# fpthink/PDGN

Measured on AMD Instinct MI355X. Metric: generator+D step points/sec (B=35, 256->2048 pts), higher is better.
Workload: dtype f32; 1 GPU; PDGNet_v2 G+D iteration (models/PDGNet_v2.py:171-256), chair-shaped synthetic batch, per-GPU batch 35, 256->2048 pts, random-init weights; global_batch=35, parallelism=dp1, losses_finite=True, hipgraph=False, issue=list

## Files before the change

### include/pdgn_hip.h

```cpp
#ifndef PDGN_HIP_H
#define PDGN_HIP_H

#include <stdint.h>

#ifdef __cplusplus
extern "C" {
#endif

#define PDGN_ERR_INVALID (-1)
#define PDGN_KNN_MAX_NSAMPLE 200

typedef void *pdgn_stream_t;

#define PDGN_ABI_VERSION 35
int pdgn_abi_version(void);

int pdgn_knnquery(int b, int n, int m, int nsample, const float *xyz, const float *new_xyz,
                  int32_t *idx, float *dist2, pdgn_stream_t stream);

int pdgn_grouping_forward(int b, int c, int n, int m, int nsample, const float *points,
                          const int32_t *idx, float *out, pdgn_stream_t stream);

int pdgn_grouping_backward(int b, int c, int n, int m, int nsample, const float *grad_out,
                           const int32_t *idx, float *grad_points, pdgn_stream_t stream);

int pdgn_nearestneighbor(int b, int n, int m, const float *unknown, const float *known,
                         float *dist2, int32_t *idx, pdgn_stream_t stream);

int pdgn_interpolation_forward(int b, int c, int m, int n, const float *points,
                               const int32_t *idx, const float *weight, float *out,
                               pdgn_stream_t stream);

int pdgn_interpolation_backward(int b, int c, int n, int m, const float *grad_out,
                                const int32_t *idx, const float *weight, float *grad_points,
                                pdgn_stream_t stream);

int pdgn_nndistance(int b, int n, const float *xyz, int m, const float *xyz2, float *result,
                    int32_t *result_i, float *result2, int32_t *result2_i, pdgn_stream_t stream);

int pdgn_nndistance_grad(int b, int n, const float *xyz1, int m, const float *xyz2,
                         const float *grad_dist1, const int32_t *idx1, const float *grad_dist2,
                         const int32_t *idx2, float *grad_xyz1, float *grad_xyz2,
                         pdgn_stream_t stream);

int pdgn_approxmatch(int b, int n, int m, const float *xyz1, const float *xyz2, float *match,
                     float *temp, pdgn_stream_t stream);

// ... 12 lines not shown

int pdgn_window_gather_sum(int b, int n, int k, int ldy, int T, int P, int C, int off, int offc,
                           const float *Y, const int32_t *idx, const float *bias, int bias_bstride,
                           float *out, pdgn_stream_t stream);
int pdgn_window_gather_sum_stats(int b, int n, int k, int ldy, int T, int P, int C, int off, int offc,
                                 const float *Y, const int32_t *idx, const float *bias, int bias_bstride,
                                 float *out, float *scratch, pdgn_stream_t stream);

int pdgn_window_gather_sum_backward(int b, int n, int k, int ldy, int T, int P, int C, int off,
                                    int offc, const float *dout, const int32_t *idx, float *dY,
                                    pdgn_stream_t stream);

int pdgn_knn_graph_transpose(int b, int n, int k, const int32_t *idx, int32_t *rowptr, int32_t *edges,
                             int32_t *scratch, pdgn_stream_t stream);
int pdgn_window_gather_sum_backward_csr(int b, int n, int k, int ldy, int T, int P, int C, int off,
                                        int offc, const float *dout, const int32_t *rowptr,
                                        const int32_t *edges, float *dY, unsigned *max_out, int max_init, pdgn_stream_t stream);

long long pdgn_bn_scratch_floats(long long rows, int c);
int pdgn_bn_stats(long long rows, int c, float eps, float momentum, const float *x, const float *gamma,
                  const float *beta, const float *pre_bias, float *running_mean, float *running_var,
                  float *scratch, float *stats, pdgn_stream_t stream);
int pdgn_bn_eval_stats(int c, float eps, const float *gamma, const float *beta, const float *pre_bias,
                       const float *running_mean, const float *running_var, float *stats,
                       pdgn_stream_t stream);
int pdgn_bn_stats_from_partials(long long rows, int c, float eps, float momentum, const float *gamma,
                                const float *beta, const float *pre_bias, float *running_mean, float *running_var,
                                const float *scratch, float *stats, pdgn_stream_t stream);
int pdgn_bn_stats_from_gemm_partials(long long rows, int c, long long nparts, int block_rows, float eps, float momentum,
                                     const float *gamma, const float *beta, const float *pre_bias,
                                     float *running_mean, float *running_var, const float *partials,
                                     float *stats, double *scratch, pdgn_stream_t stream);
long long pdgn_bn_blocks_scratch_doubles(int c, long long nparts);
int pdgn_bn_act_forward(long long rows, int c, int act, const float *x, const float *stats,
                        const float *mul, float *y, int interleave_n, pdgn_stream_t stream);
int pdgn_bn_act_backward(long long rows, int c, int act, int training, const float *x,
                         const float *dy, const float *mul, const float *stats, float *scratch,
                         float *bsums, float *dx, float *dmul, int interleave_n, pdgn_stream_t stream);

long long pdgn_bn_maxpool_scratch_floats(int b, int c);
int pdgn_bn_act_maxpool(int b, int n, int c, int act, const float *x, const float *stats, float *scratch,
                        float *ymax, int32_t *yarg, pdgn_stream_t stream);
long long pdgn_bn_stats_maxpool_scratch_floats(int b, int c);
int pdgn_bn_stats_act_maxpool(int b, int n, int c, int act, float eps, float momentum, const float *x, const float *gamma,
                              const float *beta, const float *pre_bias, float *running_mean, float *running_var, float *scratch,
                              float *stats, float *ymax, int32_t *yarg, pdgn_stream_t stream);
int pdgn_bn_act_maxpool_backward(int b, int n, int c, int act, int training, const float *x,
                                 const float *dout, const int32_t *yarg, const float *stats,
                                 float *scratch, float *bsums, float *dx, pdgn_stream_t stream);
long long pdgn_dense_bn_maxpool_backward_scratch(int b, int c, int k);
int pdgn_dense_bn_maxpool_backward(int b, int n, int c, int k, int act, const float *x, const float *dout, const int32_t *yarg,
                                   const float *stats, const float *h, int ldh, const float *W, int ldw, float *scratch,
                                   float *dh, float *dW, int lddw, float *bsums, pdgn_stream_t stream);
long long pdgn_dense_bn_maxpool_input_grad_scratch(int b, int c, int k);
int pdgn_dense_bn_maxpool_input_grad(int b, int n, int c, int k, int act, const float *x, const float *dout,
                                     const int32_t *yarg, const float *stats, const float *h, int ldh,
                                     const float *W, int ldw, float *scratch, float *dh, pdgn_stream_t stream);

int pdgn_group_colsum(long long groups, long long group_rows, int c, const float *x, long long ldx, float *out,
                      pdgn_stream_t stream);

int pdgn_softmax_slots_permute(long long m, int k, int c, const float *h, float *w, pdgn_stream_t stream);
int pdgn_bn_softmax_slots_permute(long long m, int k, int c, int act, const float *x, const float *stats,
                                  float *w, pdgn_stream_t stream);
int pdgn_bn_softmax_slots_permute_mul(long long m, int k, int c, int act, const float *x, const float *stats,
                                      int act_u, const float *u, const float *stats_u, float *w, float *y,
// ... 266 lines not shown
```

### pdgn_amd/csrc/bnact.hip

```cpp
#include "common.h"

#include "bn_geom.h"
#define ACT_NONE 0
#define ACT_RELU 1
#define ACT_LEAKY 2

__device__ __forceinline__ float act_fwd(float z, int act) {
    if (act == ACT_RELU) return fmaxf(z, 0.f);
    if (act == ACT_LEAKY) return z > 0.f ? z : 0.01f * z;
    return z;
}
__device__ __forceinline__ float act_grad(float z, int act) {
    if (act == ACT_RELU) return z > 0.f ? 1.f : 0.f;
    if (act == ACT_LEAKY) return z > 0.f ? 1.f : 0.01f;
    return 1.f;
}

struct ClGeom {
    int cg, cgb, rl;
};

__global__ __launch_bounds__(BN_THREADS) void cl_stats_kernel(long long R, int C, int cgb, int rows_per_block,
                                                              const float *__restrict__ x,
                                                              float *__restrict__ part) {
// ... 152 lines not shown
            const double mb = pv + s * inv;
            a += n * mb;
            b += (sq - s * s * inv) + n * mb * mb;
        }
    red[pl][cl] = a;
    red2[pl][cl] = b;
    __syncthreads();
    for (int h = FIN_PL / 2; h > 0; h >>= 1) {
        if (pl < h) {
            red[pl][cl] += red[pl + h][cl];
            red2[pl][cl] += red2[pl + h][cl];
        }
        __syncthreads();
    }
    if (!ok || threadIdx.x >= FIN_CH) return;
    const double mean = red[0][cl] / (double)R;
    double var = red2[0][cl] / (double)R - mean * mean;
    var = var < 0 ? 0 : var;
    const float invstd = (float)(1.0 / sqrt(var + (double)eps));
    const float g = gamma ? gamma[c] : 1.f, be = beta ? beta[c] : 0.f;
    const float scale = g * invstd;
    stats[c] = scale;
    stats[C + c] = be - (float)mean * scale;
    stats[2 * C + c] = (float)mean;
    stats[3 * C + c] = invstd;
    if (running_mean) {
        const double unbiased = R > 1 ? var * (double)R / (double)(R - 1) : var;
        const float mb = (float)mean + (pre_bias ? pre_bias[c] : 0.f);
        running_mean[c] = (1.f - momentum) * running_mean[c] + momentum * mb;
        running_var[c] = (1.f - momentum) * running_var[c] + momentum * (float)unbiased;
    }
}

__global__ __launch_bounds__(FIN_CH * FIN_PL) void cl_finalize_blocks_slice_kernel(
    long long R, int C, int nparts, int rpp, int per_slice, const float *__restrict__ part, double *__restrict__ scratch) {
    __shared__ double red[FIN_PL][FIN_CH], red2[FIN_PL][FIN_CH];
    const int cl = threadIdx.x % FIN_CH, pl = threadIdx.x / FIN_CH;
    const int c = blockIdx.x * FIN_CH + cl;
    const bool ok = c < C;
    double a = 0, b = 0;
    const double inv_full = 1.0 / (double)rpp;
    const int pmax_all = (int)min((long long)nparts, (R + rpp - 1) / rpp);
    const int p0 = blockIdx.y * per_slice, pmax = min(pmax_all, p0 + per_slice);
    if (ok)
#pragma unroll 4
        for (int p = p0 + pl; p < pmax; p += FIN_PL) {
            const long long left = R - (long long)p * rpp;
            const bool full = left >= rpp;
            const double n = (double)(full ? rpp : left), inv = full ? inv_full : 1.0 / (double)left;
            const float *q = part + (size_t)p * 3 * C + c;
            const double s = (double)q[0], sq = (double)q[C], pv = (double)q[2 * C];
            const double mb = pv + s * inv;
            a += n * mb;
            b += (sq - s * s * inv) + n * mb * mb;
        }
    red[pl][cl] = a;
    red2[pl][cl] = b;
    __syncthreads();
    for (int h = FIN_PL / 2; h > 0; h >>= 1) {
        if (pl < h) {
            red[pl][cl] += red[pl + h][cl];
            red2[pl][cl] += red2[pl + h][cl];
        }
        __syncthreads();
    }
    if (!ok || threadIdx.x >= FIN_CH) return;
// ... 38 lines not shown
    __shared__ double ra[4][64], rb[4][64];
    const int cl = threadIdx.x & 63, pl = threadIdx.x >> 6;
    const int c = blockIdx.x * 64 + cl;
    double a = 0, b = 0;
    if (c < C)
        for (int s = pl; s < slices; s += 4) {
            a += scratch[((size_t)s * 2) * C + c];
            b += scratch[((size_t)s * 2 + 1) * C + c];
        }
    ra[pl][cl] = a;
    rb[pl][cl] = b;
    __syncthreads();
    if (pl != 0 || c >= C) return;
    a = ((ra[0][cl] + ra[1][cl]) + ra[2][cl]) + ra[3][cl];
    b = ((rb[0][cl] + rb[1][cl]) + rb[2][cl]) + rb[3][cl];
    const double mean = a / (double)R;
    double var = b / (double)R - mean * mean;
    var = var < 0 ? 0 : var;
    const float invstd = (float)(1.0 / sqrt(var + (double)eps));
    const float g = gamma ? gamma[c] : 1.f, be = beta ? beta[c] : 0.f;
    const float scale = g * invstd;
    stats[c] = scale;
    stats[C + c] = be - (float)mean * scale;
    stats[2 * C + c] = (float)mean;
    stats[3 * C + c] = invstd;
    if (running_mean) {
        const double unbiased = R > 1 ? var * (double)R / (double)(R - 1) : var;
        const float mb = (float)mean + (pre_bias ? pre_bias[c] : 0.f);
        running_mean[c] = (1.f - momentum) * running_mean[c] + momentum * mb;
        running_var[c] = (1.f - momentum) * running_var[c] + momentum * (float)unbiased;
    }
}

static inline int fb_slices(int c, long long nparts) {
    if (nparts < 512) return 0;
    if (c % 64 == 0) {
        if (nparts <= 1400) return 0;
        long long s64 = nparts / 64;
        return (int)(s64 < 2 ? 2 : (s64 > 128 ? 128 : s64));
    }
    long long s = 512 / (c / 4 > 0 ? c / 4 : 1);
    s = s > 32 ? 32 : s;
    while (s > 1 && nparts / s < 128) s >>= 1;
    return s < 2 ? 0 : (int)s;
}

__global__ void cl_eval_stats_kernel(int C, float eps, const float *__restrict__ gamma, const float *__restrict__ beta,
                                     const float *__restrict__ pre_bias, const float *__restrict__ running_mean,
                                     const float *__restrict__ running_var, float *__restrict__ stats) {
    const int c = blockIdx.x * blockDim.x + threadIdx.x;
    if (c >= C) return;
    const float invstd = rsqrtf(running_var[c] + eps);
    const float g = gamma ? gamma[c] : 1.f, b = beta ? beta[c] : 0.f;
    const float m = running_mean[c] - (pre_bias ? pre_bias[c] : 0.f);
    stats[c] = g * invstd;
    stats[C + c] = b - m * g * invstd;
    stats[2 * C + c] = m;
    stats[3 * C + c] = invstd;
}

__device__ __forceinline__ void cl_interleaved_rows(long long r, int pn, long long &ra, long long &rb) {
    const long long b = r / pn;
    ra = b * 2 * pn + (r - b * pn);
    rb = ra + pn;
}

__global__ __launch_bounds__(BN_THREADS) void cl_apply_kernel(long long R, int C, int cgb, int rows_per_block, int act,
                                                              const float *__restrict__ x,
                                                              const float *__restrict__ stats,
                                                              const float *__restrict__ mul, float *__restrict__ y, int pn) {
    const int cgl = threadIdx.x % cgb, rlane = threadIdx.x / cgb, rl = BN_THREADS / cgb;
    const int cgi = blockIdx.x * cgb + cgl;
    if (cgi * 4 >= C) return;
    const long long r0 = (long long)blockIdx.y * rows_per_block;
    const long long r1 = min(R, r0 + rows_per_block);
    const float4 sc = *reinterpret_cast<const float4 *>(stats + cgi * 4);
    const float4 sh = *reinterpret_cast<const float4 *>(stats + C + cgi * 4);
// ... 183 lines not shown

extern "C" int pdgn_bn_stats(long long rows, int c, float eps, float momentum, const float *x, const float *gamma,
                             const float *beta, const float *pre_bias, float *running_mean, float *running_var,
                             float *scratch, float *stats, pdgn_stream_t stream) {
    if (rows < 1 || c < 4 || c % 4) return PDGN_ERR_INVALID;
    hipStream_t s = (hipStream_t)stream;
    int cgb, gx, gy, rpb;
    cl_geometry(rows, c, &cgb, &gx, &gy, &rpb);
    hipLaunchKernelGGL(cl_stats_kernel, dim3(gx, gy), dim3(BN_THREADS), 0, s, rows, c, cgb, rpb, x, scratch);
    hipLaunchKernelGGL(cl_finalize_kernel, dim3(cdiv(c, FIN_CH)), dim3(FIN_CH * FIN_PL), 0, s, rows, c, gy, eps, momentum, scratch,
                       gamma, beta, pre_bias, running_mean, running_var, stats, x);
    return pdgn_launch_status();
}

extern "C" int pdgn_bn_stats_from_partials(long long rows, int c, float eps, float momentum, const float *gamma,
                                           const float *beta, const float *pre_bias, float *running_mean,
                                           float *running_var, const float *scratch, float *stats, pdgn_stream_t stream) {
    if (rows < 1 || c < 4 || c % 4) return PDGN_ERR_INVALID;
    int cgb, gx, gy, rpb;
    cl_geometry(rows, c, &cgb, &gx, &gy, &rpb);
    hipLaunchKernelGGL(cl_finalize_kernel, dim3(cdiv(c, FIN_CH)), dim3(FIN_CH * FIN_PL), 0, (hipStream_t)stream, rows, c, gy, eps,
                       momentum, scratch, gamma, beta, pre_bias, running_mean, running_var, stats, (const float *)nullptr);
    return pdgn_launch_status();
}

extern "C" int pdgn_bn_stats_from_gemm_partials(long long rows, int c, long long nparts, int block_rows, float eps,
                                                float momentum, const float *gamma, const float *beta, const float *pre_bias,
                                                float *running_mean, float *running_var, const float *partials,
                                                float *stats, double *scratch, pdgn_stream_t stream) {
    if (rows < 1 || c < 4 || c % 4 || nparts < 1 || nparts > 0x7fffffffLL || block_rows < 1 ||
        nparts * (long long)block_rows < rows)
        return PDGN_ERR_INVALID;
    const int slices = scratch ? fb_slices(c, nparts) : 0;
    if (slices > 1) {
        const int per = (int)((nparts + slices - 1) / slices);
        if (c % 64 == 0)
            hipLaunchKernelGGL(cl_finalize_blocks_slice64_kernel, dim3(c / 64, slices), dim3(256), 0, (hipStream_t)stream, rows, c, (int)nparts,
                               block_rows, per, partials, scratch);
        else
            hipLaunchKernelGGL(cl_finalize_blocks_slice_kernel, dim3(cdiv(c, FIN_CH), slices), dim3(FIN_CH * FIN_PL), 0,
                               (hipStream_t)stream, rows, c, (int)nparts, block_rows, per, partials, scratch);
        hipLaunchKernelGGL(cl_finalize_blocks_join_kernel, dim3(cdiv(c, 64)), dim3(256), 0, (hipStream_t)stream, rows, c, slices,
                           eps, momentum, (const double *)scratch, gamma, beta, pre_bias, running_mean, running_var, stats);
        return pdgn_launch_status();
    }
    hipLaunchKernelGGL(cl_finalize_blocks_kernel, dim3(cdiv(c, FIN_CH)), dim3(FIN_CH * FIN_PL), 0, (hipStream_t)stream, rows, c,
                       (int)nparts, block_rows, eps, momentum, partials, gamma, beta, pre_bias, running_mean, running_var, stats);
    return pdgn_launch_status();
}

extern "C" long long pdgn_bn_blocks_scratch_doubles(int c, long long nparts) {
    if (c < 1 || nparts < 1) return PDGN_ERR_INVALID;
    return (long long)fb_slices(c, nparts) * 2 * c;
}

extern "C" int pdgn_bn_eval_stats(int c, float eps, const float *gamma, const float *beta, const float *pre_bias,
                                  const float *running_mean, const float *running_var, float *stats,
                                  pdgn_stream_t stream) {
    if (c < 1) return PDGN_ERR_INVALID;
    hipLaunchKernelGGL(cl_eval_stats_kernel, dim3(cdiv(c, 256)), dim3(256), 0, (hipStream_t)stream, c, eps, gamma,
                       beta, pre_bias, running_mean, running_var, stats);
    return pdgn_launch_status();
}

extern "C" int pdgn_bn_act_forward(long long rows, int c, int act, const float *x, const float *stats, const float *mul,
                                   float *y, int interleave_n, pdgn_stream_t stream) {
    if (rows < 1 || c < 4 || c % 4 || act < 0 || act > 2) return PDGN_ERR_INVALID;
    if (interleave_n < 0 || (interleave_n > 0 && (rows % interleave_n || mul))) return PDGN_ERR_INVALID;
    int cgb, gx, gy, rpb;
    cl_geometry(rows, c, &cgb, &gx, &gy, &rpb);
    hipLaunchKernelGGL(cl_apply_kernel, dim3(gx, gy), dim3(BN_THREADS), 0, (hipStream_t)stream, rows, c, cgb, rpb, act,
                       x, stats, mul, y, interleave_n);
    return pdgn_launch_status();
}

extern "C" int pdgn_bn_act_backward(long long rows, int c, int act, int training, const float *x, const float *dy,
                                    const float *mul, const float *stats, float *scratch, float *bsums, float *dx,
                                    float *dmul, int interleave_n, pdgn_stream_t stream) {
    if (rows < 1 || c < 4 || c % 4 || act < 0 || act > 2) return PDGN_ERR_INVALID;
    if (interleave_n < 0 || (interleave_n > 0 && (rows % interleave_n || mul))) return PDGN_ERR_INVALID;
// ... 778 lines not shown
```

### pdgn_amd/csrc/gemm_x3.hip

```cpp
#include <atomic>
#include <type_traits>

#include "gemm_shared.h"

#ifndef X3_FENCE
#define X3_FENCE 2
#endif
#ifndef X3_DEFAULT_MASK
#define X3_DEFAULT_MASK 0x000
#endif
#ifndef X3_FENCE16
#define X3_FENCE16 2
#endif
#ifndef X3_ABLATE
#define X3_ABLATE 0
#endif

typedef float f32x16 __attribute__((ext_vector_type(16)));
typedef float f32x2 __attribute__((ext_vector_type(2)));
typedef __bf16 bf16x8 __attribute__((ext_vector_type(8)));
typedef __bf16 bf16x2 __attribute__((ext_vector_type(2)));

struct X3Parts {
    u32x4 h, m, l;
// ... 17 lines not shown
__device__ __forceinline__ f32x16 x3_mfma(const u32x4 a, const u32x4 b, const f32x16 c) {
    return __builtin_amdgcn_mfma_f32_32x32x16_bf16(__builtin_bit_cast(bf16x8, a), __builtin_bit_cast(bf16x8, b), c, 0, 0, 0);
}

typedef _Float16 f16x8 __attribute__((ext_vector_type(8)));
typedef _Float16 f16x2 __attribute__((ext_vector_type(2)));
__device__ __forceinline__ unsigned x2_cvt_pk(float a, float b) {
    const f32x2 v = {a, b};
    return __builtin_bit_cast(unsigned, __builtin_convertvector(v, f16x2));
}
__device__ __forceinline__ f32x16 x2_mfma(const u32x4 a, const u32x4 b, const f32x16 c) {
    return __builtin_amdgcn_mfma_f32_32x32x16_f16(__builtin_bit_cast(f16x8, a), __builtin_bit_cast(f16x8, b), c, 0, 0, 0);
}
#ifndef X2_PRODUCTS
#define X2_PRODUCTS 3
#endif

typedef float f32x4a __attribute__((ext_vector_type(4)));
__device__ __forceinline__ f32x4a x3_mfma16(const u32x4 a, const u32x4 b, const f32x4a c) {
    return __builtin_amdgcn_mfma_f32_16x16x32_bf16(__builtin_bit_cast(bf16x8, a), __builtin_bit_cast(bf16x8, b), c, 0, 0, 0);
}

template <int MS>
__device__ __forceinline__ unsigned x3_sw(unsigned r) {
    const unsigned x = (r >> 2) & 3u;
    return MS == 32 ? x : ((0x78u >> (2u * x)) & 3u);
}

template <int CTRL, int ROW_MASK>
__device__ __forceinline__ float x3_dpp_add(float v) {
    return v + __int_as_float(__builtin_amdgcn_update_dpp(0, __float_as_int(v), CTRL, ROW_MASK, 0xf, true));
}

__device__ __forceinline__ float x3_half_wave_sum(float v) {
    v = x3_dpp_add<0x111, 0xf>(v);
    v = x3_dpp_add<0x112, 0xf>(v);
    v = x3_dpp_add<0x114, 0xf>(v);
    v = x3_dpp_add<0x118, 0xf>(v);
    return x3_dpp_add<0x142, 0xa>(v);
}

__device__ __forceinline__ float x3_row_sum(float v) {
    v = x3_dpp_add<0x111, 0xf>(v);
    v = x3_dpp_add<0x112, 0xf>(v);
    v = x3_dpp_add<0x114, 0xf>(v);
    return x3_dpp_add<0x118, 0xf>(v);
}

template <int TM, int TN, int WM, int WN, int OCC, bool ATOMIC, bool WT, bool AT, bool EPI = false, bool PW = false, int MS = 32, int NP = 3>
__global__ __launch_bounds__(64 * WM * WN, OCC) void gemm_x3_kernel(const NtArgs p) {
    static_assert(!PW || (!WT && !AT), "pre-split second operand: row-major (N x K) planes only");
    static_assert(MS == 32 || MS == 16, "matrix instruction: 32x32x16 or 16x16x32");
    static_assert(NP == 3 || (NP == 2 && MS == 32), "parts: three bf16, or two fp16 on the 32x32x16 instruction");
    constexpr int NW = WM * WN, NTH = 64 * NW, BM = 32 * TM * WM, BN = 32 * TN * WN;
    constexpr int PART_A = BM * 64, PART_W = BN * 64, STAGE = NP * (PART_A + PART_W);
    constexpr int UNT = NP == 2 ? (BM + BN) * 4 : 0;
    constexpr bool STG = OCC == 1 && !ATOMIC && !(X3_ABLATE & 128) && 2 * STAGE + NW * 4096 + UNT <= 160 * 1024;
    __shared__ __attribute__((aligned(1024))) unsigned char smem[2 * STAGE + (STG ? NW * 4096 : 0) + UNT];
    float *const untab = reinterpret_cast<float *>(smem + 2 * STAGE + (STG ? NW * 4096 : 0));

    const int tid = threadIdx.x, lane = tid & 63;
    const int wave = __builtin_amdgcn_readfirstlane(tid >> 6);
    const int wm = wave / WN, wn = wave % WN;
    const int li = MS == 32 ? lane & 31 : lane & 15, lg = MS == 32 ? lane >> 5 : lane >> 4;

    const int G = gridDim.x, pid = blockIdx.x;
    const int gq = G >> 3, gr = G & 7, xcd = pid & 7;
    const int v = xcd * gq + min(xcd, gr) + (pid >> 3);

    const int KC = p.kchunks;
    auto decode = [&](int tile, int &tm, int &tn) {
        const int per_group = NT_GROUP_M * p.tiles_n;
        const int grp = tile / per_group, r = tile - grp * per_group;
        const int first = grp * NT_GROUP_M;
        const int gsz = min(NT_GROUP_M, p.tiles_m - first);
        tn = r / gsz;
        tm = first + (r - tn * gsz);
    };
    struct Cur {
        int tile, kb, kc, ke;
        int j;
        long long f, f1;
        bool valid;
    };
    auto next_item = [&](Cur &c) {
        if (p.sk_split && (ATOMIC || p.sk_ws)) {
            const int slice = v / p.sk_split;
            c.tile = p.tile_begin + v % p.sk_split;
            c.kc = c.kb = (int)(slice * p.sk_per_wg);
            c.ke = min(KC, c.kb + (int)p.sk_per_wg);
            c.valid = c.j == 0 && c.kb < KC;
// ... 286 lines not shown
    auto read_part = [&](int st, bool isA, int part, int f) {
        read_frag(st, 0, 0, 3 * (isA ? f : FA + f) + part);
    };

    f32x16 acc[TM][TN];
#pragma unroll
    for (int a = 0; a < TM; ++a)
#pragma unroll
        for (int b = 0; b < TN; ++b)
#pragma unroll
            for (int r = 0; r < 16; ++r) acc[a][b][r] = 0.f;

    constexpr int NBB = MS == 32 ? 4 * TN : 2 * TN, NA = FA;
    auto coloff = [](int bb) { return MS == 32 ? 32 * (bb >> 2) + 8 * (bb & 3) : 16 * bb; };
    auto get4 = [&](int a, int bb) {
        const int A_ = MS == 32 ? a : a >> 1, b = MS == 32 ? bb >> 2 : bb >> 1, q = MS == 32 ? bb & 3 : 2 * (a & 1) + (bb & 1);
        return (f32x4){acc[A_][b][4 * q], acc[A_][b][4 * q + 1], acc[A_][b][4 * q + 2], acc[A_][b][4 * q + 3]};
    };
    auto set4 = [&](int a, int bb, const f32x4 x) {
        const int A_ = MS == 32 ? a : a >> 1, b = MS == 32 ? bb >> 2 : bb >> 1, q = MS == 32 ? bb & 3 : 2 * (a & 1) + (bb & 1);
        acc[A_][b][4 * q] = x[0]; acc[A_][b][4 * q + 1] = x[1]; acc[A_][b][4 * q + 2] = x[2]; acc[A_][b][4 * q + 3] = x[3];
    };
    const int ldc_eff = (!ATOMIC && p.sk_ws) ? BN : p.ldc;
    __amdgpu_buffer_rsrc_t rsC = __builtin_amdgcn_make_buffer_rsrc((void *)p.C, 0, 0, 0x00020000);
    unsigned st_off[NBB];
#pragma unroll
    for (int bb = 0; bb < NBB; ++bb) st_off[bb] = NT_OOB;
    unsigned stg_off[TN];
#pragma unroll
    for (int b = 0; b < TN; ++b) stg_off[b] = NT_OOB;
    unsigned char *const stg = smem + 2 * STAGE + wave * 4096;
    u32x4 pend[4];
    auto stage_block = [&](int a, int b) {
        int lane = __builtin_amdgcn_mbcnt_hi(~0u, __builtin_amdgcn_mbcnt_lo(~0u, 0u));
        asm volatile("" : "+v"(lane));
        const int li = MS == 32 ? lane & 31 : lane & 15, lg = MS == 32 ? lane >> 5 : lane >> 4;
        const unsigned stg_wr = (unsigned)(li * 128), stg_sw = (unsigned)(li & 7);
        const unsigned stg_rd = (unsigned)((lane >> 3) * 128 + (((lane & 7) ^ (lane >> 3)) * 16));
#pragma unroll
        for (int q = 0; q < 4; ++q) {
            if (MS == 32)
                *reinterpret_cast<u32x4 *>(stg + stg_wr + (((unsigned)(2 * q + lg) ^ stg_sw) * 16)) = __builtin_bit_cast(u32x4, get4(a, 4 * b + q));
            else
                *reinterpret_cast<u32x4 *>(stg + stg_wr + (q >> 1) * 2048 + (((unsigned)(4 * (q & 1) + lg) ^ stg_sw) * 16)) =
                    __builtin_bit_cast(u32x4, get4(2 * a + (q >> 1), 2 * b + (q & 1)));
        }
#pragma unroll
        for (int j = 0; j < 4; ++j) pend[j] = *reinterpret_cast<const u32x4 *>(stg + stg_rd + j * 1024);
    };
    auto flush_block = [&](int a, int b) {
#pragma unroll
        for (int j = 0; j < 4; ++j)
            if (!(X3_ABLATE & 4))
                __builtin_amdgcn_raw_buffer_store_b128(pend[j], rsC, stg_off[b] + (unsigned)((a * 32 + 8 * j) * ldc_eff) * 4u, 0, 0);
    };
    auto store_block = [&](int a, int b) {
        if (STG) {
            stage_block(a, b);
            flush_block(a, b);
            return;
        }
#pragma unroll
        for (int q = 0; q < 4; ++q) {
            const int ra = MS == 32 ? a : 2 * a + (q >> 1), bb = MS == 32 ? 4 * b + q : 2 * b + (q & 1);
            const unsigned off = st_off[bb] + (unsigned)(ra * FR * ldc_eff) * 4u;
            if (!(X3_ABLATE & 4)) __builtin_amdgcn_raw_buffer_store_b128(__builtin_bit_cast(u32x4, get4(ra, bb)), rsC, off, 0, 0);
        }
    };
    auto finish_item = [&]() {
        int lane = __builtin_amdgcn_mbcnt_hi(~0u, __builtin_amdgcn_mbcnt_lo(~0u, 0u));
        asm volatile("" : "+v"(lane));
        const int li = MS == 32 ? lane & 31 : lane & 15, lg = MS == 32 ? lane >> 5 : lane >> 4;
        const int mloc0 = wm * 32 * TM + li, nloc0 = wn * 32 * TN + 4 * lg;
        int tm, tn;
        decode(cp.tile, tm, tn);
        const long long m0 = (long long)tm * BM;
        const int n0 = tn * BN;
        const bool to_ws = !ATOMIC && p.sk_ws != nullptr;
        if (NP == 2) {
            if (!ATOMIC) {
                float ua[TM];
#pragma unroll
                for (int a = 0; a < TM; ++a) ua[a] = untab[mloc0 + 32 * a];
#pragma unroll
                for (int bb = 0; bb < NBB; ++bb) {
                    const f32x4 uw = *reinterpret_cast<const f32x4 *>(untab + BM + nloc0 + coloff(bb));
#pragma unroll
                    for (int a = 0; a < TM; ++a) set4(a, bb, (get4(a, bb) * ua[a]) * uw);
                }
            } else {
                const int mla = wm * 32 * TM + 4 * lg, nla = wn * 32 * TN + li;
#pragma unroll
                for (int b = 0; b < TN; ++b) {
                    const float uw = untab[BM + nla + 32 * b];
#pragma unroll
                    for (int a = 0; a < TM; ++a)
#pragma unroll
                        for (int q = 0; q < 4; ++q) {
                            const f32x4 ua4 = *reinterpret_cast<const f32x4 *>(untab + mla + 32 * a + 8 * q);
#pragma unroll
                            for (int r = 0; r < 4; ++r) acc[a][b][4 * q + r] = (acc[a][b][4 * q + r] * ua4[r]) * uw;
                        }
                }
            }
// ... 42 lines not shown
#pragma unroll
                    for (int bb = 0; bb < NBB; ++bb) {
                        const int nl = nloc0 + coloff(bb);
                        set4(a, bb, get4(a, bb) + __builtin_bit_cast(f32x4, __builtin_amdgcn_raw_buffer_load_b128(
                                                      rsR, nl < ncols ? (grp * (unsigned)p.ld_rb + n0 + nl) * 4u : NT_OOB, 0, 0)));
                    }
                }
            }
            if (EPI && p.act == 2) {
#pragma unroll
                for (int a = 0; a < TM; ++a)
#pragma unroll
                    for (int b = 0; b < TN; ++b)
#pragma unroll
                        for (int r = 0; r < 16; ++r) acc[a][b][r] = acc[a][b][r] > 0.f ? acc[a][b][r] : 0.01f * acc[a][b][r];
            }
            if (EPI && p.gate) {
                __amdgpu_buffer_rsrc_t rsG = __builtin_amdgcn_make_buffer_rsrc((void *)(p.gate + m0 * p.ldgate + n0), 0,
                                                                               (int)(mrows * p.ldgate * 4), 0x00020000);
#pragma unroll
                for (int bb = 0; bb < NBB; ++bb)
#pragma unroll
                    for (int a = 0; a < NA; ++a) {
                        const int ml = mloc0 + FR * a, nl = nloc0 + coloff(bb);
                        const f32x4 g = __builtin_bit_cast(f32x4, __builtin_amdgcn_raw_buffer_load_b128(
                                                                     rsG, nl < ncols ? (unsigned)(ml * p.ldgate + nl) * 4u : NT_OOB, 0, 0));
                        f32x4 x = get4(a, bb);
#pragma unroll
                        for (int r = 0; r < 4; ++r) x[r] *= g[r] > 0.f ? 1.f : 0.01f;
                        set4(a, bb, x);
                    }
            }
            if (p.stat_part) {
                float *P = p.stat_part + ((size_t)tm * WM + wm) * 3 * p.N;
#pragma unroll
                for (int bb = 0; bb < NBB; ++bb) {
                    float cs[4] = {0.f, 0.f, 0.f, 0.f}, cq[4] = {0.f, 0.f, 0.f, 0.f}, pv[4];
                    const f32x4 x0 = get4(0, bb);
#pragma unroll
                    for (int r = 0; r < 4; ++r) {
                        if (MS == 32) {
                            const float p0 = __int_as_float(__builtin_amdgcn_readlane(__float_as_int(x0[r]), 0));
                            const float p1 = __int_as_float(__builtin_amdgcn_readlane(__float_as_int(x0[r]), 32));
                            pv[r] = lg ? p1 : p0;
                        } else {
                            const float p0 = __int_as_float(__builtin_amdgcn_readlane(__float_as_int(x0[r]), 0));
                            const float p1 = __int_as_float(__builtin_amdgcn_readlane(__float_as_int(x0[r]), 16));
                            const float p2 = __int_as_float(__builtin_amdgcn_readlane(__float_as_int(x0[r]), 32));
                            const float p3 = __int_as_float(__builtin_amdgcn_readlane(__float_as_int(x0[r]), 48));
                            pv[r] = (lg & 2) ? ((lg & 1) ? p3 : p2) : ((lg & 1) ? p1 : p0);
                        }
                    }
#pragma unroll
                    for (int a = 0; a < NA; ++a)
                        if (mloc0 + FR * a < mrows) {
                            const f32x4 x = get4(a, bb);
#pragma unroll
                            for (int r = 0; r < 4; ++r) {
                                const float d = x[r] - pv[r];
                                cs[r] += d;
                                cq[r] = __fmaf_rn(d, d, cq[r]);
                            }
                        }
#pragma unroll
                    for (int r = 0; r < 4; ++r) {
                        cs[r] = MS == 32 ? x3_half_wave_sum(cs[r]) : x3_row_sum(cs[r]);
                        cq[r] = MS == 32 ? x3_half_wave_sum(cq[r]) : x3_row_sum(cq[r]);
                    }
                    const int nl = nloc0 + coloff(bb);
                    if (li == FR - 1 && nl < ncols) {
                        *reinterpret_cast<float4 *>(P + n0 + nl) = make_float4(cs[0], cs[1], cs[2], cs[3]);
                        *reinterpret_cast<float4 *>(P + p.N + n0 + nl) = make_float4(cq[0], cq[1], cq[2], cq[3]);
                        *reinterpret_cast<float4 *>(P + 2 * p.N + n0 + nl) = make_float4(pv[0], pv[1], pv[2], pv[3]);
                    }
                }
            }
        } else {
            const bool head = cp.kb == 0;
            const int mla = wm * 32 * TM + 4 * lg, nla = wn * 32 * TN + li;
#pragma unroll
            for (int b = 0; b < FW; ++b) {
                const int nl = nla + FR * b;
                const bool nok = nl < ncols;
                const float bz = (head && p.bias && nok) ? p.bias[n0 + nl] : 0.f;
#pragma unroll
                for (int a = 0; a < FA; ++a)
#pragma unroll
                    for (int j = 0; j < (MS == 32 ? 16 : 4); ++j) {
                        const int ml = mla + FR * a + (MS == 32 ? 8 * (j >> 2) + (j & 3) : j);
                        if (nok && ml < mrows) {
                            float o = (MS == 32 ? acc[a][b][j] : acc[a >> 1][b >> 1][4 * (2 * (a & 1) + (b & 1)) + j]) + bz;
                            if (head && p.addend) o += p.addend[(m0 + ml) * p.ldadd + n0 + nl];
                            atomicAdd(p.C + (m0 + ml) * p.ldc + n0 + nl, o);
                        }
                    }
            }
        }
    };

    constexpr int NPROD = NP == 3 ? 6 : X2_PRODUCTS;
    constexpr int SM = NPROD * TM * TN, NM = 2 * SM, NFR = NP * (TM + TN);
    constexpr int BAR = 2 * TM * TN > NFR + 2 ? 2 * TM * TN : NFR + 2;
    constexpr int CT_PER_Q = 4, NCT = NQ * CT_PER_Q;
    constexpr int C_LO = 1, C_HI = NM - BAR - 1;
    static_assert(MS == 16 || (BAR < SM && NFR + 2 <= SM), "k step too short for its fragment reads");
    auto conv_task = [&](int st, int k) {
        const int q = k / CT_PER_Q, sub = k % CT_PER_Q;
// ... 875 lines not shown
    switch (cfg) {
        case 0: return X3Big::launch<true, true>(n, k, (int)m, dY, ldy, X, ldx, nullptr, nullptr, 0, dW, k, nullptr, s, NtEpi(), dw_is_zero != 0);
        case 2: return X3Narrow::launch<true, true>(n, k, (int)m, dY, ldy, X, ldx, nullptr, nullptr, 0, dW, k, nullptr, s, NtEpi(), dw_is_zero != 0);
        default: return X3Square::launch<true, true>(n, k, (int)m, dY, ldy, X, ldx, nullptr, nullptr, 0, dW, k, nullptr, s, NtEpi(), dw_is_zero != 0);
    }
}

extern "C" long long pdgn_gemm_tn_big_workspace_floats(long long m, int n, int k) {
    if (!x3_mode() || m < 1 || n < 4 || k < 4) return 0;
    const int red = (int)(m > 0x7fffffff ? 0x7fffffff : m);
    switch (x3_pick(n, k, red, false)) {
        case 0: return X3Big::at_floats(n, k, red);
        case 2: return X3Narrow::at_floats(n, k, red);
        default: return X3Square::at_floats(n, k, red);
    }
}

extern "C" int pdgn_gemm_nt_ps_row_panel(long long m, int n, int k, int parts, int plain) {
    return (x3_mode() == 2 && parts == 2 && plain && m >= 1 && rp_takes(m, n, k)) ? 1 : 0;
}
extern "C" long long pdgn_gemm_nt_ps_stat_rows(long long m, int n, int k, int parts, int plain) {
    if (x3_mode() == 2 && parts == 2 && plain && m >= 1 && rp_takes(m, n, k)) return (m + 255) / 256;
    return pdgn_gemm_nt_stat_rows(m, n, k);
}
extern "C" int pdgn_gemm_nt_ps_stat_block_rows(long long m, int n, int k, int parts, int plain) {
    if (x3_mode() == 2 && parts == 2 && plain && m >= 1 && rp_takes(m, n, k)) return 256;
    return pdgn_gemm_nt_stat_block_rows(m, n, k);
}

extern "C" long long pdgn_gemm_nt_stat_rows(long long m, int n, int k) {
    if (!x3_mode()) return fp32_gemm_nt_stat_rows(m, n, k);
    if (m < 1 || n < 1 || k < 1) return PDGN_ERR_INVALID;
    switch (x3_pick(m, n, k, true)) {
        case 0: return (long long)cdiv(m, X3Big::BM) * 2;
        case 2: return (long long)cdiv(m, X3Narrow::BM) * 2;
        default: return (long long)cdiv(m, X3Square::BM) * 2;
    }
}

extern "C" int pdgn_gemm_nt_stat_block_rows(long long m, int n, int k) {
    if (!x3_mode()) return fp32_gemm_nt_stat_block_rows(m, n, k);
    if (m < 1 || n < 1 || k < 1) return PDGN_ERR_INVALID;
    switch (x3_pick(m, n, k, true)) {
        case 0: return X3Big::BM / 2;
        case 2: return X3Narrow::BM / 2;
        default: return X3Square::BM / 2;
    }
}

extern "C" int pdgn_gemm_nt_config(long long m, int n, int k, int with_stats) {
    if (!x3_mode()) return fp32_gemm_nt_config(m, n, k, with_stats);
    if (m < 1 || n < 1 || k < 1) return PDGN_ERR_INVALID;
    const int c = x3_pick(m, n, k, with_stats != 0);
    const bool sk = !with_stats;
    const int g = c == 0 ? X3Big::plan(m, n, k, sk).grid_sk : c == 1 ? X3Square::plan(m, n, k, sk).grid_sk
                                                                      : X3Narrow::plan(m, n, k, sk).grid_sk;
    return c + (g ? 16 : 0);
}
#endif
```

Baseline: 3.079 million points/s.

## Merge per-wave BN statistic partials in LDS inside GEMM epilogue

The GEMM epilogue now writes per-wave column sums, squared sums and pivots into shared memory. After a barrier, one wave row merges the WM wave partials with a pivot-shifted formula and writes one partial per tile instead of one per wave row. This halves the stat rows and the finalize work, at the cost of an extra barrier, extra LDS and some float-precision merging. A new 64-channel finalize kernel and a forcing knob are added, but by default the macros disable the new kernel.

```diff
diff --git a/include/pdgn_hip.h b/include/pdgn_hip.h
--- a/include/pdgn_hip.h
+++ b/include/pdgn_hip.h
@@ -12,7 +12,7 @@
 
 typedef void *pdgn_stream_t;
 
-#define PDGN_ABI_VERSION 35
+#define PDGN_ABI_VERSION 36
 int pdgn_abi_version(void);
 
 int pdgn_knnquery(int b, int n, int m, int nsample, const float *xyz, const float *new_xyz,
@@ -91,6 +91,7 @@
                                      float *running_mean, float *running_var, const float *partials,
                                      float *stats, double *scratch, pdgn_stream_t stream);
 long long pdgn_bn_blocks_scratch_doubles(int c, long long nparts);
+int pdgn_bn_set_finalize_form(int form);
 int pdgn_bn_act_forward(long long rows, int c, int act, const float *x, const float *stats,
                         const float *mul, float *y, int interleave_n, pdgn_stream_t stream);
 int pdgn_bn_act_backward(long long rows, int c, int act, int training, const float *x,
diff --git a/pdgn_amd/csrc/bnact.hip b/pdgn_amd/csrc/bnact.hip
--- a/pdgn_amd/csrc/bnact.hip
+++ b/pdgn_amd/csrc/bnact.hip
@@ -208,6 +208,57 @@
     }
 }
 
+#define FIN64_PL 16
+__global__ __launch_bounds__(64 * FIN64_PL) void cl_finalize_blocks64_kernel(
+    long long R, int C, int nparts, int rpp, float eps, float momentum, const float *__restrict__ part,
+    const float *__restrict__ gamma, const float *__restrict__ beta, const float *__restrict__ pre_bias,
+    float *__restrict__ running_mean, float *__restrict__ running_var, float *__restrict__ stats) {
+    __shared__ double red[FIN64_PL][64], red2[FIN64_PL][64];
+    const int cl = threadIdx.x & 63, pl = threadIdx.x >> 6;
+    const int c = blockIdx.x * 64 + cl;
+    double a = 0, b = 0;
+    const double inv_full = 1.0 / (double)rpp;
+    const int pmax = (int)min((long long)nparts, (R + rpp - 1) / rpp);
+#pragma unroll 4
+    for (int p = pl; p < pmax; p += FIN64_PL) {
+        const long long left = R - (long long)p * rpp;
+        const bool full = left >= rpp;
+        const double n = (double)(full ? rpp : left), inv = full ? inv_full : 1.0 / (double)left;
+        const float *q = part + (size_t)p * 3 * C + c;
+        const double s = (double)q[0], sq = (double)q[C], pv = (double)q[2 * C];
+        const double mb = pv + s * inv;
+        a += n * mb;
+        b += (sq - s * s * inv) + n * mb * mb;
+    }
+    red[pl][cl] = a;
+    red2[pl][cl] = b;
+    __syncthreads();
+    if (pl != 0) return;
+    a = red[0][cl];
+    b = red2[0][cl];
+#pragma unroll
+    for (int l = 1; l < FIN64_PL; ++l) {
+        a += red[l][cl];
+        b += red2[l][cl];
+    }
+    const double mean = a / (double)R;
+    double var = b / (double)R - mean * mean;
+    var = var < 0 ? 0 : var;
+    const float invstd = (float)(1.0 / sqrt(var + (double)eps));
+    const float g = gamma ? gamma[c] : 1.f, be = beta ? beta[c] : 0.f;
+    const float scale = g * invstd;
+    stats[c] = scale;
+    stats[C + c] = be - (float)mean * scale;
+    stats[2 * C + c] = (float)mean;
+    stats[3 * C + c] = invstd;
+    if (running_mean) {
+        const double unbiased = R > 1 ? var * (double)R / (double)(R - 1) : var;
+        const float mb = (float)mean + (pre_bias ? pre_bias[c] : 0.f);
+        running_mean[c] = (1.f - momentum) * running_mean[c] + momentum * mb;
+        running_var[c] = (1.f - momentum) * running_var[c] + momentum * (float)unbiased;
+    }
+}
+
 __global__ __launch_bounds__(FIN_CH * FIN_PL) void cl_finalize_blocks_slice_kernel(
     long long R, int C, int nparts, int rpp, int per_slice, const float *__restrict__ part, double *__restrict__ scratch) {
     __shared__ double red[FIN_PL][FIN_CH], red2[FIN_PL][FIN_CH];
@@ -312,7 +363,19 @@
     }
 }
 
+static int fb_forced = -1;
+extern "C" int pdgn_bn_set_finalize_form(int form) {
+    const int old = fb_forced;
+    if (form >= -1 && form <= 2) fb_forced = form;
+    return old;
+}
+
 static inline int fb_slices(int c, long long nparts) {
+    if (fb_forced == 0 || fb_forced == 1) return 0;
+    if (fb_forced == 2) {
+        const long long s = (nparts + 63) / 64;
+        return (int)(s > (c % 64 == 0 ? 128 : 32) ? (c % 64 == 0 ? 128 : 32) : s);
+    }
     if (nparts < 512) return 0;
     if (c % 64 == 0) {
         if (nparts <= 1400) return 0;
@@ -323,6 +386,19 @@
     s = s > 32 ? 32 : s;
     while (s > 1 && nparts / s < 128) s >>= 1;
     return s < 2 ? 0 : (int)s;
+}
+
+#ifndef FB64_MIN_PARTS
+#define FB64_MIN_PARTS 1
+#endif
+#ifndef FB64_MAX_PARTS
+#define FB64_MAX_PARTS 0
+#endif
+static inline bool fb_form64(int c, long long nparts) {
+    if (c % 64) return false;
+    if (fb_forced == 1) return true;
+    if (fb_forced == 0) return false;
+    return nparts >= FB64_MIN_PARTS && nparts <= FB64_MAX_PARTS;
 }
 
 __global__ void cl_eval_stats_kernel(int C, float eps, const float *__restrict__ gamma, const float *__restrict__ beta,
@@ -572,7 +648,7 @@
         nparts * (long long)block_rows < rows)
         return PDGN_ERR_INVALID;
     const int slices = scratch ? fb_slices(c, nparts) : 0;
-    if (slices > 1) {
+    if (slices > 1 || (slices == 1 && fb_forced == 2)) {
         const int per = (int)((nparts + slices - 1) / slices);
         if (c % 64 == 0)
             hipLaunchKernelGGL(cl_finalize_blocks_slice64_kernel, dim3(c / 64, slices), dim3(256), 0, (hipStream_t)stream, rows, c, (int)nparts,
@@ -584,8 +660,12 @@
                            eps, momentum, (const double *)scratch, gamma, beta, pre_bias, running_mean, running_var, stats);
         return pdgn_launch_status();
     }
-    hipLaunchKernelGGL(cl_finalize_blocks_kernel, dim3(cdiv(c, FIN_CH)), dim3(FIN_CH * FIN_PL), 0, (hipStream_t)stream, rows, c,
-                       (int)nparts, block_rows, eps, momentum, partials, gamma, beta, pre_bias, running_mean, running_var, stats);
+    if (fb_form64(c, nparts))
+        hipLaunchKernelGGL(cl_finalize_blocks64_kernel, dim3(c / 64), dim3(64 * FIN64_PL), 0, (hipStream_t)stream, rows, c, (int)nparts,
+                           block_rows, eps, momentum, partials, gamma, beta, pre_bias, running_mean, running_var, stats);
+    else
+        hipLaunchKernelGGL(cl_finalize_blocks_kernel, dim3(cdiv(c, FIN_CH)), dim3(FIN_CH * FIN_PL), 0, (hipStream_t)stream, rows, c,
+                           (int)nparts, block_rows, eps, momentum, partials, gamma, beta, pre_bias, running_mean, running_var, stats);
     return pdgn_launch_status();
 }
 
diff --git a/pdgn_amd/csrc/gemm_x3.hip b/pdgn_amd/csrc/gemm_x3.hip
--- a/pdgn_amd/csrc/gemm_x3.hip
+++ b/pdgn_amd/csrc/gemm_x3.hip
@@ -73,6 +73,12 @@
     return v + __int_as_float(__builtin_amdgcn_update_dpp(0, __float_as_int(v), CTRL, ROW_MASK, 0xf, true));
 }
 
+__device__ __forceinline__ int x3_lane_here() {
+    int l;
+    asm volatile("v_mbcnt_lo_u32_b32 %0, -1, 0\n\tv_mbcnt_hi_u32_b32 %0, -1, %0" : "=&v"(l));
+    return l;
+}
+
 __device__ __forceinline__ float x3_half_wave_sum(float v) {
     v = x3_dpp_add<0x111, 0xf>(v);
     v = x3_dpp_add<0x112, 0xf>(v);
@@ -97,7 +103,10 @@
     constexpr int PART_A = BM * 64, PART_W = BN * 64, STAGE = NP * (PART_A + PART_W);
     constexpr int UNT = NP == 2 ? (BM + BN) * 4 : 0;
     constexpr bool STG = OCC == 1 && !ATOMIC && !(X3_ABLATE & 128) && 2 * STAGE + NW * 4096 + UNT <= 160 * 1024;
-    __shared__ __attribute__((aligned(1024))) unsigned char smem[2 * STAGE + (STG ? NW * 4096 : 0) + UNT];
+    constexpr int STATW = 32 * TN * 3 * WM;
+    static_assert(STATW * 4 <= 4096, "the statistics table must fit a staging block");
+    constexpr int STATL = (ATOMIC || STG) ? 0 : WN * STATW * 4;
+    __shared__ __attribute__((aligned(1024))) unsigned char smem[2 * STAGE + (STG ? NW * 4096 : 0) + UNT + STATL];
     float *const untab = reinterpret_cast<float *>(smem + 2 * STAGE + (STG ? NW * 4096 : 0));
 
     const int tid = threadIdx.x, lane = tid & 63;
@@ -450,8 +459,7 @@
     unsigned char *const stg = smem + 2 * STAGE + wave * 4096;
     u32x4 pend[4];
     auto stage_block = [&](int a, int b) {
-        int lane = __builtin_amdgcn_mbcnt_hi(~0u, __builtin_amdgcn_mbcnt_lo(~0u, 0u));
-        asm volatile("" : "+v"(lane));
+        const int lane = x3_lane_here();
         const int li = MS == 32 ? lane & 31 : lane & 15, lg = MS == 32 ? lane >> 5 : lane >> 4;
         const unsigned stg_wr = (unsigned)(li * 128), stg_sw = (unsigned)(li & 7);
         const unsigned stg_rd = (unsigned)((lane >> 3) * 128 + (((lane & 7) ^ (lane >> 3)) * 16));
@@ -486,8 +494,7 @@
         }
     };
     auto finish_item = [&]() {
-        int lane = __builtin_amdgcn_mbcnt_hi(~0u, __builtin_amdgcn_mbcnt_lo(~0u, 0u));
-        asm volatile("" : "+v"(lane));
+        const int lane = x3_lane_here();
         const int li = MS == 32 ? lane & 31 : lane & 15, lg = MS == 32 ? lane >> 5 : lane >> 4;
         const int mloc0 = wm * 32 * TM + li, nloc0 = wn * 32 * TN + 4 * lg;
         int tm, tn;
@@ -596,7 +603,10 @@
                     }
             }
             if (p.stat_part) {
-                float *P = p.stat_part + ((size_t)tm * WM + wm) * 3 * p.N;
+                constexpr int WC = 32 * TN;
+                float *const ST = STG ? reinterpret_cast<float *>(smem + 2 * STAGE + wn * 4096)
+                                      : reinterpret_cast<float *>(smem + 2 * STAGE + UNT) + wn * STATW;
+                float *const SL = ST + wm * 3 * WC;
 #pragma unroll
                 for (int bb = 0; bb < NBB; ++bb) {
                     float cs[4] = {0.f, 0.f, 0.f, 0.f}, cq[4] = {0.f, 0.f, 0.f, 0.f}, pv[4];
@@ -631,12 +641,35 @@
                         cs[r] = MS == 32 ? x3_half_wave_sum(cs[r]) : x3_row_sum(cs[r]);
                         cq[r] = MS == 32 ? x3_half_wave_sum(cq[r]) : x3_row_sum(cq[r]);
                     }
-                    const int nl = nloc0 + coloff(bb);
-                    if (li == FR - 1 && nl < ncols) {
-                        *reinterpret_cast<float4 *>(P + n0 + nl) = make_float4(cs[0], cs[1], cs[2], cs[3]);
-                        *reinterpret_cast<float4 *>(P + p.N + n0 + nl) = make_float4(cq[0], cq[1], cq[2], cq[3]);
-                        *reinterpret_cast<float4 *>(P + 2 * p.N + n0 + nl) = make_float4(pv[0], pv[1], pv[2], pv[3]);
+                    const int cw = 4 * lg + coloff(bb);
+                    if (li == FR - 1) {
+                        *reinterpret_cast<float4 *>(SL + cw) = make_float4(cs[0], cs[1], cs[2], cs[3]);
+                        *reinterpret_cast<float4 *>(SL + WC + cw) = make_float4(cq[0], cq[1], cq[2], cq[3]);
+                        *reinterpret_cast<float4 *>(SL + 2 * WC + cw) = make_float4(pv[0], pv[1], pv[2], pv[3]);
                     }
+                }
+                asm volatile("s_waitcnt lgkmcnt(0)" ::: "memory");
+                __builtin_amdgcn_s_barrier();
+                asm volatile("" ::: "memory");
+                const int jl = x3_lane_here();
+                const int cn = wn * WC + jl;
+                if (wm == 0 && jl < WC && cn < ncols) {
+                    float S = ST[jl], Q = ST[WC + jl];
+                    const float pv0 = ST[2 * WC + jl];
+#pragma unroll
+                    for (int w = 1; w < WM; ++w) {
+                        const int nw = min(32 * TM, (int)mrows - w * 32 * TM);
+                        if (nw > 0) {
+                            const float Sw = ST[w * 3 * WC + jl], Qw = ST[(w * 3 + 1) * WC + jl];
+                            const float d = ST[(w * 3 + 2) * WC + jl] - pv0, fn = (float)nw;
+                            S += Sw + fn * d;
+                            Q += (Qw + 2.f * d * Sw) + fn * (d * d);
+                        }
+                    }
+                    float *P = p.stat_part + (size_t)tm * 3 * p.N + n0 + cn;
+                    P[0] = S;
+                    P[p.N] = Q;
+                    P[2 * (size_t)p.N] = pv0;
                 }
             }
         } else {
@@ -1578,9 +1611,9 @@
     if (!x3_mode()) return fp32_gemm_nt_stat_rows(m, n, k);
     if (m < 1 || n < 1 || k < 1) return PDGN_ERR_INVALID;
     switch (x3_pick(m, n, k, true)) {
-        case 0: return (long long)cdiv(m, X3Big::BM) * 2;
-        case 2: return (long long)cdiv(m, X3Narrow::BM) * 2;
-        default: return (long long)cdiv(m, X3Square::BM) * 2;
+        case 0: return (long long)cdiv(m, X3Big::BM);
+        case 2: return (long long)cdiv(m, X3Narrow::BM);
+        default: return (long long)cdiv(m, X3Square::BM);
     }
 }
 
@@ -1588,9 +1621,9 @@
     if (!x3_mode()) return fp32_gemm_nt_stat_block_rows(m, n, k);
     if (m < 1 || n < 1 || k < 1) return PDGN_ERR_INVALID;
     switch (x3_pick(m, n, k, true)) {
-        case 0: return X3Big::BM / 2;
-        case 2: return X3Narrow::BM / 2;
-        default: return X3Square::BM / 2;
+        case 0: return X3Big::BM;
+        case 2: return X3Narrow::BM;
+        default: return X3Square::BM;
     }
 }
 
```

Result: no change. 3.052 million points/s (-0.9%).
